# AmnonDrory/LidarRegistration

Hardware: AMD Instinct MI355X
Metric: registration pairs/sec (30k-pt FCGF pairs, mutual-NN + 50k RANSAC iters + refit) (higher is better)
Workload: dtype f32; 1 GPU; configs[1]: 30000-pt x32-d synthetic FCGF pair, --mode MNN --iters 50000, 3-pt sampling + ELC + LS refit; 192 distinct resident pairs per GPU, T copied to the host inside the timed region; pairs_per_batched_call=32, batched_calls_in_flight_per_gpu=2, parallelism=pair-sharded x1

## Files before the change

lidarregistration_amd/csrc/lr_api.hip:

```cpp
#include "lr_internal.h"
#include <stdarg.h>
#include <string.h>
#include <stdlib.h>
#include <new>

static thread_local char g_err[512] = "";

void lr_set_error(const char *fmt, ...)
{
    va_list ap;
    va_start(ap, fmt);
    vsnprintf(g_err, sizeof(g_err), fmt, ap);
    va_end(ap);
}

static_assert(sizeof(lr_ransac_params) == 72 && sizeof(lr_pair_params) == 112 && sizeof(lr_pair_result) == 496,
              "ABI structs changed: update include/lidarreg.h, _ext.py, INTEGRATION.md and tests/test_abi_cpu.py together");

extern "C" int lr_version(void) { return 103; }
extern "C" const char *lr_last_error(void) { return g_err; }

static inline void forget_last_batch(lr_workspace *ws) { if (ws) { ws->last_batch = 0; ws->last_T_final = nullptr; } }

static int g_fake_device = -1;
// ... 48 lines not shown
    int cur = -1;
    LR_HIP(hipGetDevice(&cur));
    if (g_fake_device >= 0) cur = g_fake_device;
    if (cur != attr.device) {
        lr_set_error("%s: the scratch lives on device %d but device %d is current (hipSetDevice / torch.cuda.set_device before the call)", who, attr.device, cur);
        return LR_EINVAL;
    }
    if (st) {
        hipDevice_t sd = -1;
        if (hipStreamGetDevice(st, &sd) == hipSuccess) {
            if ((int)sd != attr.device) { lr_set_error("%s: the stream belongs to device %d, the scratch to device %d", who, (int)sd, attr.device); return LR_EINVAL; }
        } else (void)hipGetLastError();
    }
    const lr_device_info *info = nullptr;
    LR_TRY_HIP(device_info(attr.device, &info));
    if (!info->ok) { lr_set_error("%s: device %d is %s; this library holds gfx950 code objects only", who, attr.device, info->arch); return LR_EINVAL; }
    if (n_cus) *n_cus = info->cus;
    return LR_OK;
}

extern "C" int lr_debug_fake_current_device(int device) { g_fake_device = device; return LR_OK; }

namespace {
struct Carver {
    size_t off = 0;
    char *base = nullptr;
    template <class T> T *take(size_t count)
    {
        off = (off + 255) & ~size_t(255);
        T *p = base ? reinterpret_cast<T *>(base + off) : nullptr;
        off += sizeof(T) * count;
        return p;
    }
};

void carve(lr_workspace *ws, Carver &c)
{
    const size_t n0 = ws->max_n0, n1 = ws->max_n1, n = ws->max_n, it = ws->max_iters;
    ws->nrm0 = c.take<float>(n0); ws->nrm1 = c.take<float>(n1);
    ws->H0 = c.take<_Float16>(n0 * 32); ws->H1 = c.take<_Float16>(n1 * 32);
    if (ws->dim != LR_FEAT_DIM) { ws->P0 = c.take<float>(n0 * 32); ws->P1 = c.take<float>(n1 * 32); }
    ws->tau = c.take<float>(n);
    ws->yfin = c.take<float>(n * LR_NN_MAX_STRIPS);
    ws->yshare = c.take<uint32_t>(n);
    ws->cand_cnt = c.take<int32_t>(LR_NN16_CNT_INTS(n)); ws->cand = c.take<int32_t>(LR_NN16_SEG_INTS(n));
    ws->counters = c.take<int32_t>(LR_CNT_TOTAL);
    ws->bmax0 = c.take<float>(n0 / 32 + 2); ws->bmax1 = c.take<float>(n1 / 32 + 2);
    ws->bmin0 = c.take<float>(n0 / 32 + 2); ws->bmin1 = c.take<float>(n1 / 32 + 2);
    ws->nn_range = c.take<float>(8);
    ws->rev_seed = c.take<uint32_t>(n1); ws->rev_rows = c.take<int32_t>(n1);
    ws->rev_seed64 = c.take<unsigned long long>(n1);
    ws->rev_cols = c.take<int32_t>(n0); ws->rev_s1 = c.take<float>(n0); ws->rev_pos = c.take<int32_t>(n0);
    ws->rev_tmin = c.take<float>(n0 / 32 + 2); ws->rev_hist = c.take<int32_t>(2 * 4096);
    ws->Hs = c.take<_Float16>(n0 * 32); ws->nrms = c.take<float>(n0);
    ws->nn_idx1 = c.take<int32_t>(n0); ws->nn_idx2 = c.take<int32_t>(n0);
    ws->nn_s1 = c.take<float>(n0); ws->nn_s2 = c.take<float>(n0);
    ws->rev_idx1 = c.take<int32_t>(n1);
    ws->is_bb = c.take<uint8_t>(n0);
    ws->blk_cnt = c.take<int32_t>(n0 / 256 + 2);
    ws->corr_idx0 = c.take<int32_t>(n0); ws->corr_idx1 = c.take<int32_t>(n0); ws->corr_idx2 = c.take<int32_t>(n0);
    ws->corr_score = c.take<float>(n0);
    ws->ratio = c.take<float>(n0);
    ws->cell = c.take<int32_t>(n0); ws->cell_sorted = c.take<int32_t>(n0);
    ws->gpf_quota = c.take<double>(LR_GPF_MAX_CELLS);
    ws->gpf_cells = c.take<int32_t>(3 * (LR_GPF_MAX_CELLS + 8) > 2 * (LR_PR_BUCKETS + 8) + 8 ? 3 * (LR_GPF_MAX_CELLS + 8) : 2 * (LR_PR_BUCKETS + 8) + 8);
    ws->gpf_keep = c.take<uint8_t>(n0);
    ws->gpf_f = c.take<float>(8);
    ws->corr8 = c.take<float>((n0 + 2) * 8);
    ws->prosac_G = c.take<int32_t>(n0 + 2); ws->prosac_rank = c.take<int32_t>(n0);
    ws->models = c.take<float>(it * 12);
    ws->models64 = c.take<double>(it * 12);
    ws->model_h = c.take<int32_t>(it);
    ws->models2 = c.take<float>(it * 12); ws->models64_2 = c.take<double>(it * 12); ws->model_h2 = c.take<int32_t>(it);
    ws->score_cnt = c.take<uint32_t>(it);
    ws->score_ssq = c.take<unsigned long long>(it);
    ws->refit_part = c.take<double>((n0 / 256 + 2) * 16);
    ws->icp_ints = c.take<int32_t>(3 * (32768 + 8));
    ws->icp_bucket = c.take<int32_t>(n1); ws->icp_pts = c.take<float>(4 * n1);
    ws->icp_state = c.take<double>(32); ws->icp_part = c.take<double>((n0 / 256 + 2) * 18);
    ws->lo_list = c.take<int32_t>(n0);
    ws->lo_ctl = c.take<char>(LR_LO_CTL_BYTES);
    ws->sc_info = c.take<char>(LR_SC_INFO_BYTES);
    ws->corr8s = c.take<float>((n0 + 4) * 8);
    ws->sc_perm = c.take<int32_t>(it); ws->sc_glen = c.take<int32_t>(it / 64 + 2);
    ws->sc_mb = c.take<uint8_t>(it); ws->sc_cb = c.take<uint8_t>(n0);
    ws->models_s = c.take<float>(it * 12);
    ws->res_tmp = c.take<lr_ransac_result>(1);
    ws->T_tmp = c.take<double>(48);
}
}

extern "C" int lr_workspace_create(lr_workspace **out, int max_n0, int max_n1, int dim, int max_iters)
{
    return lr_workspace_create_batch(out, 1, max_n0, max_n1, dim, max_iters);
}

extern "C" int lr_workspace_create_batch(lr_workspace **out, int max_pairs, int max_n0, int max_n1, int dim, int max_iters)
{
    LR_REQUIRE(out, LR_EINVAL, "lr_workspace_create: null output");
    LR_REQUIRE(max_pairs >= 1 && max_pairs <= LR_MAX_BATCH, LR_EINVAL, "lr_workspace_create_batch: max_pairs must be in [1, 64]");
    LR_REQUIRE(max_n0 > 0 && max_n1 > 0 && max_iters >= 0, LR_EINVAL, "lr_workspace_create: sizes must be positive");
    LR_REQUIRE(dim >= 1 && dim <= LR_FEAT_DIM, LR_EINVAL, "lr_workspace_create: descriptors of 1 to 32 dimensions are supported");
    LR_REQUIRE(max_n0 < (1 << 22) && max_n1 < (1 << 22), LR_ESIZE, "lr_workspace_create: clouds are limited to 2^22 points");
    int dev = -1;
    LR_HIP(hipGetDevice(&dev));
    const lr_device_info *di = nullptr;
    LR_TRY_HIP(device_info(dev, &di));
    if (!di->ok) {
        lr_set_error("lr_workspace_create: device %d is %s; this library holds gfx950 (MI355X) code objects only", dev, di->arch);
        return LR_EINVAL;
    }
    lr_workspace *ws = new (std::nothrow) lr_workspace();
    LR_REQUIRE(ws, LR_ENOMEM, "lr_workspace_create: host allocation failed");
    memset(ws, 0, sizeof(*ws));
    ws->device = dev; ws->n_cus = di->cus;
    ws->max_n0 = max_n0; ws->max_n1 = max_n1; ws->max_n = max_n0 > max_n1 ? max_n0 : max_n1;
    ws->dim = dim; ws->max_iters = max_iters > 0 ? max_iters : 1;
    ws->max_pairs = max_pairs;
    ws->nn_blocks_target = 3 * ws->n_cus;
    ws->nn_blocks_batch = 12 * ws->n_cus;
    ws->nn_sample_stride = 0; ws->rev_strips = 0; ws->nn_second_auto = 0; ws->clock_probe = 0;
    Carver sizing;
    carve(ws, sizing);
    ws->stride = (sizing.off + 511) & ~size_t(255);
    const size_t desc_off = ws->stride * (size_t)max_pairs;
    const size_t clk_off = (desc_off + sizeof(lr_pair_desc) * LR_MAX_BATCH + 255) & ~size_t(255);
    ws->bytes = clk_off + 256;
    hipError_t e = hipMalloc(&ws->base, ws->bytes);
    if (e != hipSuccess) {
        lr_set_error("lr_workspace_create: hipMalloc(%zu) -> %s", ws->bytes, hipGetErrorString(e));
        delete ws;
        return e == hipErrorOutOfMemory ? LR_ENOMEM : LR_EHIP;
    }
    Carver real;
    real.base = ws->base;
    carve(ws, real);
    ws->descs = reinterpret_cast<lr_pair_desc *>(ws->base + desc_off);
    ws->clk_dev = reinterpret_cast<unsigned long long *>(ws->base + clk_off);
    if (hipHostMalloc(reinterpret_cast<void **>(&ws->form_host), 2 * sizeof(int32_t), hipHostMallocMapped) == hipSuccess) {
        ws->form_host[0] = ws->form_host[1] = 0;
        if (hipHostGetDevicePointer(reinterpret_cast<void **>(&ws->form_dev), ws->form_host, 0) != hipSuccess) { (void)hipHostFree(ws->form_host); ws->form_host = ws->form_dev = nullptr; }
    } else { (void)hipGetLastError(); ws->form_host = ws->form_dev = nullptr; }
    if (hipMemset(ws->base, 0, ws->bytes) != hipSuccess || hipStreamSynchronize(nullptr) != hipSuccess) {
        if (ws->form_host) (void)hipHostFree(ws->form_host);
        (void)hipFree(ws->base); delete ws; lr_set_error("lr_workspace_create: hipMemset failed"); return LR_EHIP;
    }
    for (int k = 0; k < LR_NEV; ++k)
        if (hipEventCreate(&ws->timer.ev[k]) != hipSuccess) {
            for (int q = 0; q < k; ++q) (void)hipEventDestroy(ws->timer.ev[q]);
            if (ws->form_host) (void)hipHostFree(ws->form_host);
            (void)hipFree(ws->base); delete ws; lr_set_error("lr_workspace_create: hipEventCreate failed"); return LR_EHIP;
        }
    *out = ws;
    return LR_OK;
}

extern "C" int lr_workspace_destroy(lr_workspace *ws)
{
    if (!ws) return LR_OK;
    if (ws->form_host) (void)hipHostFree(ws->form_host);
    for (int k = 0; k < LR_NEV; ++k) (void)hipEventDestroy(ws->timer.ev[k]);
    (void)hipFree(ws->base);
    delete ws;
    return LR_OK;
}

extern "C" size_t lr_workspace_bytes(const lr_workspace *ws) { return ws ? ws->bytes : 0; }

// ... 473 lines not shown
```

lidarregistration_amd/csrc/lr_internal.h:

```cpp
#pragma once
#include <hip/hip_runtime.h>
#include <stdint.h>
#include <stdio.h>
#include "../../include/lidarreg.h"

void lr_set_error(const char *fmt, ...);

#define LR_HIP(call)                                                                      \
    do {                                                                                  \
        hipError_t e_ = (call);                                                           \
        if (e_ != hipSuccess) {                                                           \
            lr_set_error("%s:%d: %s -> %s", __FILE__, __LINE__, #call, hipGetErrorString(e_)); \
            return LR_EHIP;                                                               \
        }                                                                                 \
    } while (0)

#define LR_LAUNCH_CHECK() LR_HIP(hipGetLastError())

#define LR_REQUIRE(cond, code, msg)                 \
    do {                                            \
        if (!(cond)) { lr_set_error("%s", msg); return code; } \
    } while (0)

#define LR_NN16_SEG 4096
// ... 59 lines not shown
    int on;
    unsigned recorded;
    int n_samples;
    hipEvent_t ev[LR_NEV];
    struct { float call, fwd, fwd_filter, rev_filter, ransac, rev, nn; } ms;
    bool has(lr_event e) const { return (recorded >> e & 1u) != 0; }
    bool begun() const { return has(LR_EV_FWD_FILTER_END); }
    bool armed() const { return on && !begun(); }
};

struct lr_workspace {
    int max_n0, max_n1, max_n, dim, max_iters;
    int max_pairs;
    int device, n_cus;
    int last_npairs;
    int last_batch;
    int last_mx0, last_mx1;
    const double *last_T_final;
    hipStream_t last_stream;
    size_t stride;
    size_t bytes;
    char *base;
    lr_pair_desc *descs;
    float *nrm0, *nrm1;
    _Float16 *H0, *H1;
    float *P0, *P1;
    float *tau;
    uint32_t *yshare;
    float *yfin;
    int32_t *cand_cnt, *cand;
    float *bmax0, *bmax1;
    float *bmin0, *bmin1;
    float *nn_range;
    int form_prev[2];
    int32_t *form_host, *form_dev;
    uint32_t *rev_seed;
    unsigned long long *rev_seed64;
    int32_t *rev_rows;
    int32_t *rev_cols;
    int32_t *rev_pos;
    float *rev_s1;
    float *rev_tmin;
    int32_t *rev_hist;
    _Float16 *Hs; float *nrms;
    int nn_blocks_target;
    int nn_blocks_batch;
    int nn_sample_stride;
    int rev_strips;
    int nn_second_auto;
    int clock_probe;
    unsigned long long *clk_dev;
    int32_t *counters;
    int32_t *nn_idx1, *nn_idx2;
    float *nn_s1, *nn_s2;
    int32_t *rev_idx1;
    uint8_t *is_bb;
    int32_t *blk_cnt;
    int32_t *corr_idx0, *corr_idx1, *corr_idx2;
    float *corr_score;
    float *ratio;
    int32_t *cell;
    int32_t *cell_sorted;
    double *gpf_quota;
    int32_t *gpf_cells;
    uint8_t *gpf_keep;
    float *gpf_f;
    int32_t *prosac_G;
    int32_t *prosac_rank;
    float *corr8;
    float *models;
    double *models64;
    int32_t *model_h;
    float *models2; double *models64_2; int32_t *model_h2;
    uint32_t *score_cnt;
    unsigned long long *score_ssq;
    double *refit_part;
    int32_t *lo_list;
    void *lo_ctl;
    void *sc_info;
    float *corr8s;
    int32_t *sc_perm;
    float *models_s;
    int32_t *sc_glen;
    uint8_t *sc_mb, *sc_cb;
    lr_ransac_result *res_tmp;
    double *T_tmp;
    int32_t *icp_ints;
    int32_t *icp_bucket;
    float *icp_pts;
    double *icp_state, *icp_part;
    lr_stage_timer timer;
};

struct lr_call {
    lr_workspace *ws;
    hipStream_t st;
    int pairs;
    lr_zargs z;
    bool armed;
};
static inline lr_call lr_call_single(lr_workspace *ws, void *stream) { return lr_call{ ws, (hipStream_t)stream, 1, lr_zargs{ 0, nullptr }, ws->timer.armed() }; }
static inline lr_call lr_call_batch(lr_workspace *ws, void *stream, int pairs) { return lr_call{ ws, (hipStream_t)stream, pairs, lr_zargs{ ws->stride, ws->descs }, ws->timer.armed() }; }

enum {
    LR_CNT_FIX = 0,
    LR_CNT_FIX_TOTAL,
    LR_CNT_NCORR,
    LR_CNT_NVALID,
    LR_CNT_NBB,
    LR_CNT_NREV,
    LR_CNT_RLO,
    LR_CNT_RHI,
    LR_CNT_REFIT_TICKET,
    LR_CNT_NVALID2,
    LR_CNT_FORM_MISS_F,
    LR_CNT_FORM_MISS_R,
    LR_CNT_NREFIT = 14,
    LR_CNT_COUNT = 16,
    LR_CNT_TOTAL = 64
};

__host__ __device__ inline size_t lr_corr_at(int c, int k) { return (size_t)(c >> 1) * 16 + 2 * k + (c & 1); }

struct lr_ransac_state {
    double T[12];
    unsigned long long ssq;
    long long n_valid, n_ids;
    uint32_t cnt;
    int32_t h;
    int32_t done;
    int32_t lo_pending;
    int32_t lo_calls;
    int32_t lo_timeouts;
    double sprt_eps, sprt_delta;
    unsigned long long rej_inl, rej_pts;
    unsigned long long evals, evals_full;
};
static_assert(sizeof(lr_ransac_state) <= (LR_CNT_TOTAL - LR_CNT_COUNT) * sizeof(int32_t), "lr_ransac_state does not fit");

int lr_zero_scratch(const lr_call &c, void *p, size_t bytes);
int lr_check_memory_device(const void *mem, hipStream_t st, const char *who, int *n_cus);
int lr_timer_mark(const lr_call &c, lr_event e);

int lr_nn16_prep(const lr_call &c, const float *F0, int n0, const float *F1, int n1, bool zero_counters = false);
int lr_nn16_run(const lr_call &c, const float *F0, int n0, const float *F1, int n1,
                int32_t *idx1, int32_t *idx2, float *s1, float *s2, bool seed_reverse = false);
int lr_nn16_reverse(const lr_call &c, const float *F0, int n0, const float *F1, int n1, const int32_t *fwd_idx1, int32_t *rev, bool seeded = false);

int lr_mutual_run(const lr_call &c, int n0, const int32_t *idx1, const int32_t *idx2, const int32_t *rev,
                  uint8_t *is_bb, int32_t *o0, int32_t *o1, int32_t *o2, int32_t *n_out,
                  const float *xyz0 = nullptr, const float *xyz1 = nullptr, float *corr8 = nullptr);
int lr_identity_corr(const lr_call &c, int n0, const int32_t *idx1, const int32_t *idx2,
                     int32_t *o0, int32_t *o1, int32_t *o2, int32_t *n_out);
int lr_pack_corr(const lr_call &c, const float *xyz0, const float *xyz1, const int32_t *i0, const int32_t *i1, int m_max,
                 const int32_t *m_dev, float *corr8, const int32_t *rank = nullptr);
int lr_prosac_order(const lr_call &c, const float *F0, const float *F1, int dim, const float *quality, int m_max, const int32_t *m_dev);
struct lr_gpf_subset { const int32_t *mb_dev, *b0; int32_t *has_score; double max_matches; };
int lr_gpf_run(const lr_call &c, const float *F0, int n0, const float *F1, int dim,
               const int32_t *idx1, const int32_t *idx2, const uint8_t *is_bb, const float *xyz0,
               int grid_wid, double factor, int32_t *o0, int32_t *o1, int32_t *o2, float *oscore,
               int32_t *n_out, const float *xyz1 = nullptr, float *corr8 = nullptr, const lr_gpf_subset *sub = nullptr);

int lr_icp_run(const lr_call &c, const float *xyz0, int n0, const float *xyz1, int n1, const double *T_init,
               const lr_ransac_result *gate, double max_dist, int max_iter, double rel_fit, double rel_rmse,
               double *T_out, lr_icp_result *res);

int lr_ransac_run(const lr_call &c, const float *corr8, int m_max, const int32_t *m_dev, const lr_ransac_params *p,
// ... 13 lines not shown
```

lidarregistration_amd/csrc/lr_ransac_dev.h:

```cpp
#pragma once
#include "lr_internal.h"
#include <math.h>

__device__ __forceinline__ void philox4x32_10(uint32_t c[4], uint32_t k0, uint32_t k1)
{
#pragma unroll
    for (int r = 0; r < 10; ++r) {
        uint32_t hi0 = __umulhi(0xD2511F53u, c[0]), lo0 = 0xD2511F53u * c[0];
        uint32_t hi1 = __umulhi(0xCD9E8D57u, c[2]), lo1 = 0xCD9E8D57u * c[2];
        uint32_t n0 = hi1 ^ c[1] ^ k0, n2 = hi0 ^ c[3] ^ k1;
        c[0] = n0; c[1] = lo1; c[2] = n2; c[3] = lo0;
        k0 += 0x9E3779B9u; k1 += 0xBB67AE85u;
    }
}

#include "lr_contract.h"

typedef float f32x2 __attribute__((ext_vector_type(2)));
typedef float f32x4 __attribute__((ext_vector_type(4)));

struct lr_model12 { float Rt[12]; };
__device__ __forceinline__ lr_model12 lr_load_model(const float *__restrict__ mp, size_t ms)
{
    lr_model12 M;
#pragma unroll
    for (int k = 0; k < 12; ++k) M.Rt[k] = mp[k * ms];
    return M;
}
__device__ __forceinline__ void lr_store_model(float *__restrict__ mp, size_t ms, const lr_model12 &M)
{
#pragma unroll
    for (int k = 0; k < 12; ++k) mp[k * ms] = M.Rt[k];
}
__device__ __forceinline__ float lr_corr_d2(const float Rt[12], const float *__restrict__ corr8, int i)
{
    return lr_score_d2(Rt, corr8[lr_corr_at(i, 0)], corr8[lr_corr_at(i, 1)], corr8[lr_corr_at(i, 2)], corr8[lr_corr_at(i, 3)],
                       corr8[lr_corr_at(i, 4)], corr8[lr_corr_at(i, 5)]);
}

struct lr_model12x2 {
    f32x2 c[12];
    template <class T>
    __device__ __forceinline__ explicit lr_model12x2(const T *Rt)
    {
#pragma unroll
        for (int k = 0; k < 12; ++k) { const float v = (float)Rt[k]; c[k] = f32x2{ v, v }; }
    }
};
__device__ __forceinline__ f32x2 lr_d2x2(const lr_model12x2 &S, const f32x2 px, const f32x2 py, const f32x2 pz, const f32x2 qx, const f32x2 qy, const f32x2 qz)
{
    const f32x2 x = __builtin_elementwise_fma(S.c[0], px, __builtin_elementwise_fma(S.c[1], py, __builtin_elementwise_fma(S.c[2], pz, S.c[3])));
    const f32x2 y = __builtin_elementwise_fma(S.c[4], px, __builtin_elementwise_fma(S.c[5], py, __builtin_elementwise_fma(S.c[6], pz, S.c[7])));
    const f32x2 z = __builtin_elementwise_fma(S.c[8], px, __builtin_elementwise_fma(S.c[9], py, __builtin_elementwise_fma(S.c[10], pz, S.c[11])));
    const f32x2 dx = x - qx, dy = y - qy, dz = z - qz;
    return __builtin_elementwise_fma(dx, dx, __builtin_elementwise_fma(dy, dy, dz * dz));
}
__device__ __forceinline__ f32x2 lr_d2x2(const lr_model12x2 &S, const f32x2 *o) { return lr_d2x2(S, o[0], o[1], o[2], o[3], o[4], o[5]); }
__device__ __forceinline__ void lr_record_operands(const f32x4 A, const f32x4 B, const f32x4 C, f32x2 (&o)[6])
{
    o[0] = f32x2{ A.x, A.y }; o[1] = f32x2{ A.z, A.w }; o[2] = f32x2{ B.x, B.y }; o[3] = f32x2{ B.z, B.w }; o[4] = f32x2{ C.x, C.y }; o[5] = f32x2{ C.z, C.w };
}
template <class Q>
__device__ __forceinline__ void lr_add_pair(const f32x2 d2, bool in0, bool in1, uint32_t &cnt, Q &q)
{
    const f32x2 fx = d2 * f32x2{ LR_SCORE_SCALE, LR_SCORE_SCALE };
    cnt += (in0 ? 1u : 0u) + (in1 ? 1u : 0u);
    q += (Q)(in0 ? (uint32_t)fx.x : 0u) + (Q)(in1 ? (uint32_t)fx.y : 0u);
}

#define LR_SC_HEAD 256
#define LR_SC_NB 128
#define LR_SC_W 0.0625f
#define LR_SC_MIN_M 2048
#define LR_SC_MIN_V 128
#define LR_SC_MIN_PAIRS 4
struct lr_score_info {
    unsigned long long pilot_key;
    int32_t prune;
    int32_t n_sorted;
    uint32_t box[6];
    int32_t bad;
    int32_t pad;
    int32_t hist[LR_SC_NB];
    int32_t fill[LR_SC_NB];
    int32_t offs[LR_SC_NB + 1];
};
__device__ __forceinline__ uint32_t lr_ford(float f) { const uint32_t u = __float_as_uint(f); return (u & 0x80000000u) ? ~u : (u | 0x80000000u); }
__device__ __forceinline__ float lr_ford_inv(uint32_t u) { return __uint_as_float((u & 0x80000000u) ? (u & 0x7fffffffu) : ~u); }
static_assert(sizeof(lr_score_info) <= LR_SC_INFO_BYTES, "lr_score_info does not fit its scratch block");

__device__ __forceinline__ void lr_score_info_reset(lr_score_info *info)
{
    const int t = threadIdx.x;
    if (t < LR_SC_NB) info->hist[t] = 0;
    if (t < 3) { info->box[t] = 0xffffffffu; info->box[3 + t] = 0u; }
    if (t == 0) { info->pilot_key = 0ull; info->bad = 0; info->prune = 0; }
}
__device__ __forceinline__ int lr_sc_head(int m, int V) { return (m >= LR_SC_MIN_M && V >= LR_SC_MIN_V) ? LR_SC_HEAD : 0; }

__device__ __forceinline__ void lr_sprt_redesign(lr_ransac_state *state, uint32_t nc, int mm)
{
    double eps = state->sprt_eps > 0.0 ? state->sprt_eps : LR_SPRT_EPS0, delta = state->sprt_delta > 0.0 ? state->sprt_delta : LR_SPRT_DELTA0;
    if (nc > 0) { const double e = (double)nc / (double)mm; if (e > eps && e < 1.0) eps = e; }
    if (state->rej_pts > 0) {
        const double d = (double)state->rej_inl / (double)state->rej_pts;
        if (d > 0.0 && d < 0.9 * eps && fabs(d - delta) > 0.05 * delta) delta = d;
    }
    if (!(delta < 0.9 * eps)) delta = 0.9 * eps * 0.5;
    state->sprt_eps = eps; state->sprt_delta = delta;
}

#define LO_CHUNK_REC 384
#define LO_JOBS 16
struct lr_lo_job { int32_t next_chunk, done_chunks, nchunks, pad0;
                   float Rt[LR_LO_TRIALS][12]; unsigned cnt[LR_LO_TRIALS]; unsigned long long ssq[LR_LO_TRIALS]; };
struct lr_lo_ctl { int32_t phase, pad[3]; lr_lo_job job[LO_JOBS]; };
static_assert(sizeof(lr_lo_ctl) <= LR_LO_CTL_BYTES, "lr_lo_ctl does not fit its scratch block");
```

lidarregistration_amd/csrc/lr_score.hip:

```cpp
#include "lr_ransac_dev.h"
#define LR_INF_F __builtin_huge_valf()

#ifndef LR_SCORE_CHUNK
#define LR_SCORE_CHUNK 256
#endif

__device__ __forceinline__ void lr_score_stream(const float *__restrict__ corr8, int begin, int end, int sub, float thr2,
                                                const lr_model12 &M, uint32_t &cnt, unsigned long long &ssq)
{
    const lr_model12x2 S(M.Rt);
    uint32_t q32 = 0;
    auto pair_of = [&](const f32x2 px, const f32x2 py, const f32x2 pz, const f32x2 qx, const f32x2 qy, const f32x2 qz) {
        const f32x2 d2 = lr_d2x2(S, px, py, pz, qx, qy, qz);
        const f32x2 fx = d2 * f32x2{ LR_SCORE_SCALE, LR_SCORE_SCALE };
        const bool in0 = d2.x < thr2, in1 = d2.y < thr2;
        cnt += (in0 ? 1u : 0u) + (in1 ? 1u : 0u);
        q32 += (in0 ? (uint32_t)fx.x : 0u) + (in1 ? (uint32_t)fx.y : 0u);
    };
    const int pend = end & ~1;
    for (int b0 = begin; b0 < pend; b0 += sub) {
        const int b1 = min(pend, b0 + sub);
        q32 = 0;
        int i = b0;
        const f32x2 *rec = reinterpret_cast<const f32x2 *>(corr8);
        if (i + 4 <= b1) {
            f32x2 c0[6], c1[6], n0[6], n1[6];
            auto load2 = [&](int at, f32x2 (&r0)[6], f32x2 (&r1)[6]) {
#pragma unroll
                for (int k = 0; k < 6; ++k) { r0[k] = rec[(size_t)(at >> 1) * 8 + k]; r1[k] = rec[(size_t)(at >> 1) * 8 + 8 + k]; }
                __builtin_amdgcn_sched_barrier(0);
            };
            load2(i, c0, c1);
            while (i + 4 <= b1) {
                __builtin_amdgcn_s_waitcnt(0xC07F);
                load2(i + 8 <= b1 ? i + 4 : i, n0, n1);
                pair_of(c0[0], c0[1], c0[2], c0[3], c0[4], c0[5]);
                pair_of(c1[0], c1[1], c1[2], c1[3], c1[4], c1[5]);
                i += 4;
                if (i + 4 > b1) break;
                __builtin_amdgcn_s_waitcnt(0xC07F);
                load2(i + 8 <= b1 ? i + 4 : i, c0, c1);
                pair_of(n0[0], n0[1], n0[2], n0[3], n0[4], n0[5]);
                pair_of(n1[0], n1[1], n1[2], n1[3], n1[4], n1[5]);
                i += 4;
            }
        }
        if (i < b1) {
            const f32x2 *q = rec + (size_t)(i >> 1) * 8;
            pair_of(q[0], q[1], q[2], q[3], q[4], q[5]);
        }
        ssq += q32;
    }
    if (pend < end && begin < end) {
        const float d2 = lr_corr_d2(M.Rt, corr8, pend);
        if (d2 < thr2) { cnt += 1u; ssq += lr_score_term(d2); }
    }
}

template <int HEAD>
__global__ void __launch_bounds__(256)
ransac_score_kernel(const float *__restrict__ corr8, const float *__restrict__ corr8s, int m_max, const int32_t *__restrict__ m_dev, float thr2,
                    const float *__restrict__ models, const float *__restrict__ models_s, uint32_t *__restrict__ score_cnt,
                    unsigned long long *__restrict__ score_ssq, const int32_t *__restrict__ counters, lr_score_info *__restrict__ info,
                    const int32_t *__restrict__ perm, const int32_t *__restrict__ glen, int sub, int model_stride, int vslot,
                    int gx, int total, int allow_prune, lr_zargs z)
{
    int logical;
    if (!lr_xcd_block(total, logical)) return;
    const int bxi = logical % gx, pair = logical / gx;
    lr_z(corr8, z, pair); lr_z(corr8s, z, pair); lr_z(m_dev, z, pair); lr_z(models, z, pair); lr_z(models_s, z, pair); lr_z(score_cnt, z, pair); lr_z(score_ssq, z, pair);
    lr_z(counters, z, pair); lr_z(info, z, pair); lr_z(perm, z, pair); lr_z(glen, z, pair);
    const int m = m_dev ? min(*m_dev, m_max) : m_max;
    const int V = counters[vslot];
    const int hb = (V + 63) >> 6;
    if (hb == 0 || m <= 0 || reinterpret_cast<const lr_ransac_state *>(counters + LR_CNT_COUNT)->done) return;
    const int K0 = allow_prune ? lr_sc_head(m, V) : 0;
    const int lane = threadIdx.x & 63;
    const size_t ms = (size_t)model_stride;
    const int W = gx * 4, w0 = bxi * 4 + __builtin_amdgcn_readfirstlane((int)threadIdx.x >> 6);
    if (HEAD) {
        if (K0 == 0) return;
        constexpr int HQ = 4, QL = LR_SC_HEAD / HQ;
        for (int w = w0; w < hb * HQ; w += W) {
            const int g = w % hb, qi = w / hb;
            const int slot = g * 64 + lane;
            const bool active = slot < V;
            const lr_model12 M = lr_load_model(models + (active ? slot : 0), ms);
            uint32_t cnt = 0; unsigned long long ssq = 0;
            lr_score_stream(corr8, qi * QL, (qi + 1) * QL, sub, thr2, M, cnt, ssq);
            if (active && cnt) { atomicAdd(&score_cnt[slot], cnt); atomicAdd(&score_ssq[slot], ssq); }
            if (qi == 0) {
                unsigned long long key = active ? ((unsigned long long)cnt << 32) | (unsigned long long)(0xffffffffu - (uint32_t)slot) : 0ull;
#pragma unroll
                for (int o = 32; o >= 1; o >>= 1) { const unsigned long long k2 = __shfl_xor(key, o); key = k2 > key ? k2 : key; }
                if (lane == 0) atomicMax(&info->pilot_key, key);
            }
        }
        return;
    }
    const bool prune = K0 > 0;
    const float *__restrict__ stream = prune ? corr8s : corr8;
    const int L = prune ? m - K0 : m;
    int chunks = W / hb;
    const int cmax = L / LR_SCORE_CHUNK > 0 ? L / LR_SCORE_CHUNK : 1;
    if (chunks > cmax) chunks = cmax;
    if (chunks < 1) chunks = 1;
    const int per = ((L + chunks - 1) / chunks + 1) & ~1;
    for (int w = w0; w < hb * chunks; w += W) {
        const int g = w % hb, c = w / hb;
        const int len = prune ? min(glen[g], (L + 1) & ~1) : L;
        const int begin = c * per, end = min(len, begin + per);
        if (begin >= end) continue;
        const int spos = g * 64 + lane;
        const bool active = spos < V;
        const lr_model12 M = lr_load_model((prune ? models_s : models) + (active ? spos : 0), ms);
        uint32_t cnt = 0;
        unsigned long long ssq = 0;
        lr_score_stream(stream, begin, end, sub, thr2, M, cnt, ssq);
        if (active && cnt) {
            const int slot = prune ? perm[spos] : spos;
            atomicAdd(&score_cnt[slot], cnt); atomicAdd(&score_ssq[slot], ssq);
        }
    }
}

__global__ void __launch_bounds__(256)
ransac_resid_kernel(const float *__restrict__ corr8, int m_max, const int32_t *__restrict__ m_dev, const float *__restrict__ models,
                    const int32_t *__restrict__ counters, lr_score_info *__restrict__ info, uint8_t *__restrict__ cb, int model_stride, int vslot, lr_zargs z)
{
    __shared__ int s_h[LR_SC_NB];
    __shared__ float s_red[4][6];
    __shared__ int s_bad;
    lr_z(corr8, z, blockIdx.z); lr_z(m_dev, z, blockIdx.z); lr_z(models, z, blockIdx.z); lr_z(counters, z, blockIdx.z); lr_z(info, z, blockIdx.z); lr_z(cb, z, blockIdx.z);
    const int m = m_dev ? min(*m_dev, m_max) : m_max;
    const int V = counters[vslot];
    const int tid = threadIdx.x, lane = tid & 63, wave = tid >> 6;
    const int c = blockIdx.x * 256 + tid;
    if (V <= 0 || blockIdx.x * 256 >= m || reinterpret_cast<const lr_ransac_state *>(counters + LR_CNT_COUNT)->done) return;
    const int K0 = lr_sc_head(m, V);
    if (K0 == 0) return;
    if (tid < LR_SC_NB) s_h[tid] = 0;
    if (tid == 0) s_bad = 0;
    __syncthreads();
    int ps = (int)(0xffffffffu - (uint32_t)info->pilot_key);
    ps = min(max(ps, 0), V - 1);
    const lr_model12 P = lr_load_model(models + ps, (size_t)model_stride);
    float lo[3] = { 3.0e38f, 3.0e38f, 3.0e38f }, hi[3] = { -3.0e38f, -3.0e38f, -3.0e38f };
    if (c < m) {
        bool bad = false;
#pragma unroll
        for (int a = 0; a < 3; ++a) { const float v = corr8[lr_corr_at(c, a)]; bad |= !(fabsf(v) < 3.0e38f); lo[a] = v; hi[a] = v; }
        if (bad) s_bad = 1;
        if (c >= K0) {
            constexpr float INVW = 1.0f / LR_SC_W, RMAX = LR_SC_NB * LR_SC_W;
            const float r = sqrtf(lr_corr_d2(P.Rt, corr8, c));
            int b = LR_SC_NB - 1;
            if (r < RMAX) b = min((int)(r * INVW), LR_SC_NB - 1);
            cb[c] = (uint8_t)b;
            atomicAdd(&s_h[b], 1);
        }
    }
#pragma unroll
    for (int a = 0; a < 3; ++a)
#pragma unroll
        for (int o = 32; o >= 1; o >>= 1) { lo[a] = fminf(lo[a], __shfl_xor(lo[a], o)); hi[a] = fmaxf(hi[a], __shfl_xor(hi[a], o)); }
    if (lane == 0) { for (int a = 0; a < 3; ++a) { s_red[wave][a] = lo[a]; s_red[wave][3 + a] = hi[a]; } }
    __syncthreads();
    if (tid < LR_SC_NB && s_h[tid]) atomicAdd(&info->hist[tid], s_h[tid]);
    if (tid < 6) {
        float v = s_red[0][tid];
        for (int w = 1; w < 4; ++w) v = tid < 3 ? fminf(v, s_red[w][tid]) : fmaxf(v, s_red[w][tid]);
        if (tid < 3) atomicMin(&info->box[tid], lr_ford(v)); else atomicMax(&info->box[tid], lr_ford(v));
    }
    if (tid == 0 && s_bad) info->bad = 1;
}

__global__ void __launch_bounds__(1024)
ransac_order_kernel(int m_max, const int32_t *__restrict__ m_dev, float thr2, const float *__restrict__ models, int32_t *__restrict__ counters,
                    lr_score_info *__restrict__ info, int32_t *__restrict__ perm, int32_t *__restrict__ glen, uint8_t *__restrict__ mb,
                    float *__restrict__ models_s, int model_stride, int vslot, lr_zargs z)
{
    __shared__ int s_h[LR_SC_NB], s_off[LR_SC_NB + 1], s_fill[LR_SC_NB];
    __shared__ unsigned long long s_ev[16];
    lr_z(m_dev, z, blockIdx.z); lr_z(models, z, blockIdx.z); lr_z(counters, z, blockIdx.z); lr_z(models_s, z, blockIdx.z);
    lr_z(info, z, blockIdx.z); lr_z(perm, z, blockIdx.z); lr_z(glen, z, blockIdx.z); lr_z(mb, z, blockIdx.z);
    lr_ransac_state *state = reinterpret_cast<lr_ransac_state *>(counters + LR_CNT_COUNT);
    const int m = m_dev ? min(*m_dev, m_max) : m_max;
    const int V = counters[vslot];
    const int tid = threadIdx.x, lane = tid & 63, wave = tid >> 6;
    if (V <= 0 || m <= 0 || state->done) return;
    const int K0 = lr_sc_head(m, V);
    if (K0 == 0) return;
    const size_t ms = (size_t)model_stride;
    int ps = (int)(0xffffffffu - (uint32_t)info->pilot_key);
    ps = min(max(ps, 0), V - 1);
    const lr_model12 P = lr_load_model(models + ps, ms);
    if (tid < 64) {
        const int h0 = info->hist[2 * tid], h1 = info->hist[2 * tid + 1];
        int inc = h0 + h1;
#pragma unroll
        for (int o = 1; o < 64; o <<= 1) { const int v = __shfl_up(inc, o); if (tid >= o) inc += v; }
        const int ex = inc - (h0 + h1);
        s_off[2 * tid] = ex; s_off[2 * tid + 1] = ex + h0;
        info->offs[2 * tid] = ex; info->offs[2 * tid + 1] = ex + h0;
        info->fill[2 * tid] = ex; info->fill[2 * tid + 1] = ex + h0;
        if (tid == 63) { s_off[LR_SC_NB] = inc; info->offs[LR_SC_NB] = inc; }
    }
    if (tid < LR_SC_NB) s_h[tid] = 0;
    __syncthreads();
    const float b0 = lr_ford_inv(info->box[0]), b1 = lr_ford_inv(info->box[1]), b2 = lr_ford_inv(info->box[2]);
    const float b3 = lr_ford_inv(info->box[3]), b4 = lr_ford_inv(info->box[4]), b5 = lr_ford_inv(info->box[5]);
    const float cx = 0.5f * (b0 + b3), cy = 0.5f * (b1 + b4), cz = 0.5f * (b2 + b5);
    const float ex = b3 - b0, ey = b4 - b1, ez = b5 - b2;
    float rho = 0.5f * sqrtf(ex * ex + ey * ey + ez * ez) * 1.0001f + 1e-6f;
    if (info->bad) rho = LR_INF_F;
    const float amax = fmaxf(fmaxf(fmaxf(fabsf(b0), fabsf(b3)), fmaxf(fabsf(b1), fabsf(b4))), fmaxf(fabsf(b2), fabsf(b5)));
    constexpr float INVW = 1.0f / LR_SC_W, RMAX = LR_SC_NB * LR_SC_W;
    const float thr = sqrtf(thr2);
    const float *Pm = P.Rt;
    const float pt1 = fabsf(Pm[3]) + fabsf(Pm[7]) + fabsf(Pm[11]);
    for (int v = tid; v < V; v += 1024) {
        const lr_model12 M = lr_load_model(models + v, ms);
        const float *Mm = M.Rt;
        const float d00 = Mm[0] - Pm[0], d01 = Mm[1] - Pm[1], d02 = Mm[2] - Pm[2], d10 = Mm[4] - Pm[4], d11 = Mm[5] - Pm[5], d12 = Mm[6] - Pm[6],
                    d20 = Mm[8] - Pm[8], d21 = Mm[9] - Pm[9], d22 = Mm[10] - Pm[10];
        const float F = sqrtf(d00 * d00 + d01 * d01 + d02 * d02 + d10 * d10 + d11 * d11 + d12 * d12 + d20 * d20 + d21 * d21 + d22 * d22);
        const float ux = d00 * cx + d01 * cy + d02 * cz + (Mm[3] - Pm[3]), uy = d10 * cx + d11 * cy + d12 * cz + (Mm[7] - Pm[7]),
                    uz = d20 * cx + d21 * cy + d22 * cz + (Mm[11] - Pm[11]);
        const float eps = (F * rho + sqrtf(ux * ux + uy * uy + uz * uz)) * 1.001f;
        const float slack = 0.01f + 4e-6f * (3.0f * amax + pt1 + fabsf(Mm[3]) + fabsf(Mm[7]) + fabsf(Mm[11]));
        const float cut = thr + eps + slack;
        int bv = LR_SC_NB - 1;
        if (cut < RMAX) bv = min((int)(cut * INVW), LR_SC_NB - 1);
        mb[v] = (uint8_t)bv;
        atomicAdd(&s_h[LR_SC_NB - 1 - bv], 1);
    }
    __syncthreads();
    if (tid < 64) {
        const int h0 = s_h[2 * tid], h1 = s_h[2 * tid + 1];
        int inc = h0 + h1;
#pragma unroll
        for (int o = 1; o < 64; o <<= 1) { const int v = __shfl_up(inc, o); if (tid >= o) inc += v; }
        s_fill[2 * tid] = inc - (h0 + h1); s_fill[2 * tid + 1] = inc - h1;
    }
    __syncthreads();
    for (int v = tid; v < V; v += 1024) {
        const int pos = atomicAdd(&s_fill[LR_SC_NB - 1 - (int)mb[v]], 1);
        perm[pos] = v;
#pragma unroll
        for (int k = 0; k < 12; ++k) models_s[(size_t)k * ms + pos] = models[(size_t)k * ms + v];
    }
    __syncthreads();
    const int L = m - K0;
    const int hb = (V + 63) >> 6;
    unsigned long long ev = 0;
    for (int g = tid; g < hb; g += 1024) {
        const int len = (s_off[(int)mb[perm[g * 64]] + 1] + 1) & ~1;
        glen[g] = len;
        ev += (unsigned long long)min(len, L) * (unsigned long long)min(64, V - g * 64);
    }
#pragma unroll
    for (int o = 32; o >= 1; o >>= 1) ev += __shfl_xor(ev, o);
    if (lane == 0) s_ev[wave] = ev;
    __syncthreads();
    if (tid == 0) {
        for (int w = 1; w < 16; ++w) ev += s_ev[w];
        state->evals += ev + (unsigned long long)V * (unsigned long long)K0;
        state->evals_full += (unsigned long long)V * (unsigned long long)m;
        info->prune = 1; info->n_sorted = L;
    }
}

__global__ void __launch_bounds__(256)
ransac_scatter_kernel(const float *__restrict__ corr8, float *__restrict__ corr8s, int m_max, const int32_t *__restrict__ m_dev,
                      const int32_t *__restrict__ counters, lr_score_info *__restrict__ info, const uint8_t *__restrict__ cb, int vslot, lr_zargs z)
{
    __shared__ int s_h[LR_SC_NB], s_base[LR_SC_NB];
    lr_z(corr8, z, blockIdx.z); lr_z(corr8s, z, blockIdx.z); lr_z(m_dev, z, blockIdx.z); lr_z(counters, z, blockIdx.z); lr_z(info, z, blockIdx.z); lr_z(cb, z, blockIdx.z);
    const int m = m_dev ? min(*m_dev, m_max) : m_max;
    const int V = counters[vslot];
    const int tid = threadIdx.x;
    const int c = blockIdx.x * 256 + tid;
    if (V <= 0 || blockIdx.x * 256 >= m || reinterpret_cast<const lr_ransac_state *>(counters + LR_CNT_COUNT)->done) return;
    const int K0 = lr_sc_head(m, V);
    if (K0 == 0) return;
    if (tid < LR_SC_NB) s_h[tid] = 0;
    __syncthreads();
    const bool live = c >= K0 && c < m;
    const int b = live ? (int)cb[c] : 0;
    int rank = 0;
    if (live) rank = atomicAdd(&s_h[b], 1);
    __syncthreads();
    if (tid < LR_SC_NB && s_h[tid]) s_base[tid] = atomicAdd(&info->fill[tid], s_h[tid]);
    __syncthreads();
    if (live) {
        const int pos = s_base[b] + rank;
#pragma unroll
        for (int k = 0; k < 6; ++k) corr8s[lr_corr_at(pos, k)] = corr8[lr_corr_at(c, k)];
    }
    const int L = m - K0;
    if (blockIdx.x == 0 && tid == 0 && (L & 1)) {
#pragma unroll
        for (int k = 0; k < 6; ++k) corr8s[lr_corr_at(L, k)] = k < 3 ? 0.0f : 3.0e38f;
    }
}

void lr_score_run(const lr_call &c, const float *corr8, int m_max, const int32_t *m_dev, float thr2, const float *models, int h_count, int vslot)
{
    lr_workspace *ws = c.ws; hipStream_t st = c.st;
    lr_score_info *info = reinterpret_cast<lr_score_info *>(ws->sc_info);
    int sub = (int)((4294967296.0 / (double)LR_SCORE_SCALE - 1.0) / ((double)thr2 * 1.0000001 + 1e-6));
    if (sub > 4096) sub = 4096;
    sub &= ~1;
    if (sub < 2) sub = 2;
    const bool may_prune = m_max >= LR_SC_MIN_M && h_count >= 2048 && c.pairs > LR_SC_MIN_PAIRS;
    if (may_prune) {
        const int hgx = 64, htotal = hgx * c.pairs;
        hipLaunchKernelGGL(ransac_score_kernel<1>, dim3(8 * lr_cdiv(htotal, 8)), dim3(256), 0, st, corr8, (const float *)ws->corr8s, m_max, m_dev, thr2,
                           models, (const float *)ws->models_s, ws->score_cnt, ws->score_ssq, ws->counters, info, (const int32_t *)ws->sc_perm, (const int32_t *)ws->sc_glen, sub,
                           ws->max_iters, vslot, hgx, htotal, 1, c.z);
        const dim3 cgrid(lr_cdiv(m_max, 256), 1, c.pairs);
        hipLaunchKernelGGL(ransac_resid_kernel, cgrid, dim3(256), 0, st, corr8, m_max, m_dev, models, (const int32_t *)ws->counters, info, ws->sc_cb,
                           ws->max_iters, vslot, c.z);
        hipLaunchKernelGGL(ransac_order_kernel, dim3(1, 1, c.pairs), dim3(1024), 0, st, m_max, m_dev, thr2, models, ws->counters, info,
                           ws->sc_perm, ws->sc_glen, ws->sc_mb, ws->models_s, ws->max_iters, vslot, c.z);
        hipLaunchKernelGGL(ransac_scatter_kernel, cgrid, dim3(256), 0, st, corr8, ws->corr8s, m_max, m_dev, (const int32_t *)ws->counters, info,
                           (const uint8_t *)ws->sc_cb, vslot, c.z);
    }
    const int sgx = LR_SCORE_BLOCKS / 4, stotal = sgx * c.pairs;
    hipLaunchKernelGGL(ransac_score_kernel<0>, dim3(8 * lr_cdiv(stotal, 8)), dim3(256), 0, st, corr8, (const float *)ws->corr8s, m_max, m_dev, thr2,
                       models, (const float *)ws->models_s, ws->score_cnt, ws->score_ssq, ws->counters, info, (const int32_t *)ws->sc_perm, (const int32_t *)ws->sc_glen, sub,
                       ws->max_iters, vslot, sgx, stotal, may_prune ? 1 : 0, c.z);
}
```

Baseline: 12350 pairs/s.

## Add lower-bound residual pruning to skip sorted correspondences per hypothesis group

Computes, for each RANSAC hypothesis, a lower bound on the residual of correspondences relative to a pivot model, using a rotation-axis projection. Hypotheses are ordered by a (upper bin, lower bin) class via a block exclusive scan, and each 64-hypothesis group records a start offset as well as an end offset into the residual-sorted correspondences. The score kernel then evaluates only the window between those offsets and splits it into chunks. This is meant to skip correspondences that provably cannot be inliers, at the cost of extra per-model math, a larger shared histogram, and more complex ordering.

```diff
diff --git a/lidarregistration_amd/csrc/lr_api.hip b/lidarregistration_amd/csrc/lr_api.hip
--- a/lidarregistration_amd/csrc/lr_api.hip
+++ b/lidarregistration_amd/csrc/lr_api.hip
@@ -154,8 +154,9 @@
     ws->lo_ctl = c.take<char>(LR_LO_CTL_BYTES);
     ws->sc_info = c.take<char>(LR_SC_INFO_BYTES);
     ws->corr8s = c.take<float>((n0 + 4) * 8);
-    ws->sc_perm = c.take<int32_t>(it); ws->sc_glen = c.take<int32_t>(it / 64 + 2);
+    ws->sc_perm = c.take<int32_t>(it); ws->sc_glen = c.take<int32_t>(2 * (it / 64 + 2));
     ws->sc_mb = c.take<uint8_t>(it); ws->sc_cb = c.take<uint8_t>(n0);
+    ws->sc_ml = c.take<uint8_t>(it);
     ws->models_s = c.take<float>(it * 12);
     ws->res_tmp = c.take<lr_ransac_result>(1);
     ws->T_tmp = c.take<double>(48);
diff --git a/lidarregistration_amd/csrc/lr_internal.h b/lidarregistration_amd/csrc/lr_internal.h
--- a/lidarregistration_amd/csrc/lr_internal.h
+++ b/lidarregistration_amd/csrc/lr_internal.h
@@ -165,7 +165,7 @@
     int32_t *sc_perm;
     float *models_s;
     int32_t *sc_glen;
-    uint8_t *sc_mb, *sc_cb;
+    uint8_t *sc_mb, *sc_ml, *sc_cb;
     lr_ransac_result *res_tmp;
     double *T_tmp;
     int32_t *icp_ints;
diff --git a/lidarregistration_amd/csrc/lr_ransac_dev.h b/lidarregistration_amd/csrc/lr_ransac_dev.h
--- a/lidarregistration_amd/csrc/lr_ransac_dev.h
+++ b/lidarregistration_amd/csrc/lr_ransac_dev.h
@@ -98,6 +98,22 @@
 }
 __device__ __forceinline__ int lr_sc_head(int m, int V) { return (m >= LR_SC_MIN_M && V >= LR_SC_MIN_V) ? LR_SC_HEAD : 0; }
 
+__device__ __forceinline__ float lr_sc_dmin(const float *P, const float *M, const float d[9], float ux, float uy, float uz, float rho)
+{
+    const float q21 = P[2] * M[1] + P[6] * M[5] + P[10] * M[9], q12 = P[1] * M[2] + P[5] * M[6] + P[9] * M[10];
+    const float q02 = P[0] * M[2] + P[4] * M[6] + P[8] * M[10], q20 = P[2] * M[0] + P[6] * M[4] + P[10] * M[8];
+    const float q10 = P[1] * M[0] + P[5] * M[4] + P[9] * M[8], q01 = P[0] * M[1] + P[4] * M[5] + P[8] * M[9];
+    float ax = q21 - q12, ay = q02 - q20, az = q10 - q01;
+    const float n2 = ax * ax + ay * ay + az * az;
+    if (n2 > 1e-12f) { const float n = sqrtf(n2); ax = ax / n; ay = ay / n; az = az / n; }
+    else { ax = 0.0f; ay = 0.0f; az = 1.0f; }
+    const float bx = P[0] * ax + P[1] * ay + P[2] * az, by = P[4] * ax + P[5] * ay + P[6] * az, bz = P[8] * ax + P[9] * ay + P[10] * az;
+    const float nb = sqrtf(bx * bx + by * by + bz * bz);
+    const float g0 = d[0] * bx + d[3] * by + d[6] * bz, g1 = d[1] * bx + d[4] * by + d[7] * bz, g2 = d[2] * bx + d[5] * by + d[8] * bz;
+    const float num = fabsf(bx * ux + by * uy + bz * uz) - sqrtf(g0 * g0 + g1 * g1 + g2 * g2) * rho * 1.001f;
+    return num / (nb * 1.001f);
+}
+
 __device__ __forceinline__ void lr_sprt_redesign(lr_ransac_state *state, uint32_t nc, int mm)
 {
     double eps = state->sprt_eps > 0.0 ? state->sprt_eps : LR_SPRT_EPS0, delta = state->sprt_delta > 0.0 ? state->sprt_delta : LR_SPRT_DELTA0;
diff --git a/lidarregistration_amd/csrc/lr_score.hip b/lidarregistration_amd/csrc/lr_score.hip
--- a/lidarregistration_amd/csrc/lr_score.hip
+++ b/lidarregistration_amd/csrc/lr_score.hip
@@ -1,4 +1,5 @@
 #include "lr_ransac_dev.h"
+#include "lr_prims.h"
 #define LR_INF_F __builtin_huge_valf()
 
 #ifndef LR_SCORE_CHUNK
@@ -108,8 +109,15 @@
     const int per = ((L + chunks - 1) / chunks + 1) & ~1;
     for (int w = w0; w < hb * chunks; w += W) {
         const int g = w % hb, c = w / hb;
-        const int len = prune ? min(glen[g], (L + 1) & ~1) : L;
-        const int begin = c * per, end = min(len, begin + per);
+        int first = 0, len = L, gper = per;
+        if (prune) {
+            first = glen[2 * g]; len = min(glen[2 * g + 1], (L + 1) & ~1);
+            const int range = len - first;
+            const int gc = min(chunks, max(range / LR_SCORE_CHUNK, 1));
+            if (c >= gc) continue;
+            gper = ((range + gc - 1) / gc + 1) & ~1;
+        }
+        const int begin = first + c * gper, end = min(len, begin + gper);
         if (begin >= end) continue;
         const int spos = g * 64 + lane;
         const bool active = spos < V;
@@ -175,15 +183,22 @@
     if (tid == 0 && s_bad) info->bad = 1;
 }
 
+#define LR_SC_TRI (LR_SC_NB * (LR_SC_NB + 1) / 2)
+__device__ __forceinline__ int lr_sc_class(int hi, int lo)
+{
+    const int h = LR_SC_NB - 1 - hi;
+    return h * LR_SC_NB - ((h * (h - 1)) >> 1) + lo;
+}
 __global__ void __launch_bounds__(1024)
 ransac_order_kernel(int m_max, const int32_t *__restrict__ m_dev, float thr2, const float *__restrict__ models, int32_t *__restrict__ counters,
-                    lr_score_info *__restrict__ info, int32_t *__restrict__ perm, int32_t *__restrict__ glen, uint8_t *__restrict__ mb,
-                    float *__restrict__ models_s, int model_stride, int vslot, lr_zargs z)
-{
-    __shared__ int s_h[LR_SC_NB], s_off[LR_SC_NB + 1], s_fill[LR_SC_NB];
+                    lr_score_info *__restrict__ info, int32_t *__restrict__ perm, int32_t *__restrict__ glen,
+                    uint8_t *__restrict__ mb, uint8_t *__restrict__ ml, float *__restrict__ models_s, int model_stride, int vslot, lr_zargs z)
+{
+    __shared__ int s_off[LR_SC_NB + 1], s_cls[LR_SC_TRI];
+    __shared__ int s_gmin[1024];
     __shared__ unsigned long long s_ev[16];
     lr_z(m_dev, z, blockIdx.z); lr_z(models, z, blockIdx.z); lr_z(counters, z, blockIdx.z); lr_z(models_s, z, blockIdx.z);
-    lr_z(info, z, blockIdx.z); lr_z(perm, z, blockIdx.z); lr_z(glen, z, blockIdx.z); lr_z(mb, z, blockIdx.z);
+    lr_z(info, z, blockIdx.z); lr_z(perm, z, blockIdx.z); lr_z(glen, z, blockIdx.z); lr_z(mb, z, blockIdx.z); lr_z(ml, z, blockIdx.z);
     lr_ransac_state *state = reinterpret_cast<lr_ransac_state *>(counters + LR_CNT_COUNT);
     const int m = m_dev ? min(*m_dev, m_max) : m_max;
     const int V = counters[vslot];
@@ -206,14 +221,16 @@
         info->fill[2 * tid] = ex; info->fill[2 * tid + 1] = ex + h0;
         if (tid == 63) { s_off[LR_SC_NB] = inc; info->offs[LR_SC_NB] = inc; }
     }
-    if (tid < LR_SC_NB) s_h[tid] = 0;
+    for (int k = tid; k < LR_SC_TRI; k += 1024) s_cls[k] = 0;
+    s_gmin[tid] = LR_SC_NB - 1;
     __syncthreads();
     const float b0 = lr_ford_inv(info->box[0]), b1 = lr_ford_inv(info->box[1]), b2 = lr_ford_inv(info->box[2]);
     const float b3 = lr_ford_inv(info->box[3]), b4 = lr_ford_inv(info->box[4]), b5 = lr_ford_inv(info->box[5]);
     const float cx = 0.5f * (b0 + b3), cy = 0.5f * (b1 + b4), cz = 0.5f * (b2 + b5);
     const float ex = b3 - b0, ey = b4 - b1, ez = b5 - b2;
     float rho = 0.5f * sqrtf(ex * ex + ey * ey + ez * ez) * 1.0001f + 1e-6f;
-    if (info->bad) rho = LR_INF_F;
+    const bool bad = info->bad != 0;
+    if (bad) rho = LR_INF_F;
     const float amax = fmaxf(fmaxf(fmaxf(fabsf(b0), fabsf(b3)), fmaxf(fabsf(b1), fabsf(b4))), fmaxf(fabsf(b2), fabsf(b5)));
     constexpr float INVW = 1.0f / LR_SC_W, RMAX = LR_SC_NB * LR_SC_W;
     const float thr = sqrtf(thr2);
@@ -222,31 +239,31 @@
     for (int v = tid; v < V; v += 1024) {
         const lr_model12 M = lr_load_model(models + v, ms);
         const float *Mm = M.Rt;
-        const float d00 = Mm[0] - Pm[0], d01 = Mm[1] - Pm[1], d02 = Mm[2] - Pm[2], d10 = Mm[4] - Pm[4], d11 = Mm[5] - Pm[5], d12 = Mm[6] - Pm[6],
-                    d20 = Mm[8] - Pm[8], d21 = Mm[9] - Pm[9], d22 = Mm[10] - Pm[10];
-        const float F = sqrtf(d00 * d00 + d01 * d01 + d02 * d02 + d10 * d10 + d11 * d11 + d12 * d12 + d20 * d20 + d21 * d21 + d22 * d22);
-        const float ux = d00 * cx + d01 * cy + d02 * cz + (Mm[3] - Pm[3]), uy = d10 * cx + d11 * cy + d12 * cz + (Mm[7] - Pm[7]),
-                    uz = d20 * cx + d21 * cy + d22 * cz + (Mm[11] - Pm[11]);
+        const float d[9] = { Mm[0] - Pm[0], Mm[1] - Pm[1], Mm[2] - Pm[2], Mm[4] - Pm[4], Mm[5] - Pm[5], Mm[6] - Pm[6],
+                             Mm[8] - Pm[8], Mm[9] - Pm[9], Mm[10] - Pm[10] };
+        const float F = sqrtf(d[0] * d[0] + d[1] * d[1] + d[2] * d[2] + d[3] * d[3] + d[4] * d[4] + d[5] * d[5] + d[6] * d[6] + d[7] * d[7] + d[8] * d[8]);
+        const float ux = d[0] * cx + d[1] * cy + d[2] * cz + (Mm[3] - Pm[3]), uy = d[3] * cx + d[4] * cy + d[5] * cz + (Mm[7] - Pm[7]),
+                    uz = d[6] * cx + d[7] * cy + d[8] * cz + (Mm[11] - Pm[11]);
         const float eps = (F * rho + sqrtf(ux * ux + uy * uy + uz * uz)) * 1.001f;
         const float slack = 0.01f + 4e-6f * (3.0f * amax + pt1 + fabsf(Mm[3]) + fabsf(Mm[7]) + fabsf(Mm[11]));
         const float cut = thr + eps + slack;
         int bv = LR_SC_NB - 1;
         if (cut < RMAX) bv = min((int)(cut * INVW), LR_SC_NB - 1);
-        mb[v] = (uint8_t)bv;
-        atomicAdd(&s_h[LR_SC_NB - 1 - bv], 1);
-    }
-    __syncthreads();
-    if (tid < 64) {
-        const int h0 = s_h[2 * tid], h1 = s_h[2 * tid + 1];
-        int inc = h0 + h1;
-#pragma unroll
-        for (int o = 1; o < 64; o <<= 1) { const int v = __shfl_up(inc, o); if (tid >= o) inc += v; }
-        s_fill[2 * tid] = inc - (h0 + h1); s_fill[2 * tid + 1] = inc - h1;
-    }
+        const float lcut = lr_sc_dmin(Pm, Mm, d, ux, uy, uz, rho) - thr - slack;
+        int lv = 0;
+        if (!bad && lcut > 0.0f && lcut < 3.0e38f) lv = lcut < RMAX ? min((int)(lcut * INVW), LR_SC_NB - 1) : LR_SC_NB - 1;
+        lv = min(lv, bv);
+        mb[v] = (uint8_t)bv; ml[v] = (uint8_t)lv;
+        atomicAdd(&s_cls[lr_sc_class(bv, lv)], 1);
+    }
+    __syncthreads();
+    lr_block_exscan(s_cls, LR_SC_TRI);
     __syncthreads();
     for (int v = tid; v < V; v += 1024) {
-        const int pos = atomicAdd(&s_fill[LR_SC_NB - 1 - (int)mb[v]], 1);
+        const int lv = (int)ml[v];
+        const int pos = atomicAdd(&s_cls[lr_sc_class((int)mb[v], lv)], 1);
         perm[pos] = v;
+        if ((pos >> 6) < 1024) atomicMin(&s_gmin[pos >> 6], lv);
 #pragma unroll
         for (int k = 0; k < 12; ++k) models_s[(size_t)k * ms + pos] = models[(size_t)k * ms + v];
     }
@@ -255,9 +272,11 @@
     const int hb = (V + 63) >> 6;
     unsigned long long ev = 0;
     for (int g = tid; g < hb; g += 1024) {
+        const int n = min(64, V - g * 64);
         const int len = (s_off[(int)mb[perm[g * 64]] + 1] + 1) & ~1;
-        glen[g] = len;
-        ev += (unsigned long long)min(len, L) * (unsigned long long)min(64, V - g * 64);
+        const int beg = g < 1024 ? s_off[s_gmin[g]] & ~1 : 0;
+        glen[2 * g] = beg; glen[2 * g + 1] = len;
+        ev += (unsigned long long)max(min(len, L) - beg, 0) * (unsigned long long)n;
     }
 #pragma unroll
     for (int o = 32; o >= 1; o >>= 1) ev += __shfl_xor(ev, o);
@@ -323,7 +342,7 @@
         hipLaunchKernelGGL(ransac_resid_kernel, cgrid, dim3(256), 0, st, corr8, m_max, m_dev, models, (const int32_t *)ws->counters, info, ws->sc_cb,
                            ws->max_iters, vslot, c.z);
         hipLaunchKernelGGL(ransac_order_kernel, dim3(1, 1, c.pairs), dim3(1024), 0, st, m_max, m_dev, thr2, models, ws->counters, info,
-                           ws->sc_perm, ws->sc_glen, ws->sc_mb, ws->models_s, ws->max_iters, vslot, c.z);
+                           ws->sc_perm, ws->sc_glen, ws->sc_mb, ws->sc_ml, ws->models_s, ws->max_iters, vslot, c.z);
         hipLaunchKernelGGL(ransac_scatter_kernel, cgrid, dim3(256), 0, st, corr8, ws->corr8s, m_max, m_dev, (const int32_t *)ws->counters, info,
                            (const uint8_t *)ws->sc_cb, vslot, c.z);
     }
```

Result: slower. 12200 pairs/s (-1.2%).
